# NVIDIA/nvidia-resiliency-ext

Hardware: AMD Instinct MI355X
Metric: generate_report_latency_us (lower is better)
Workload: dtype f32; 1 GPU; 8 ranks x 64 sections x 10000 samples per report, ring capacity 10000, relative+individual scores, gather_on_rank0; logical_ranks_per_gpu=8, rows_per_gpu=512, exchange=none (single process)

## Files before the change

### include/nvrx_straggler.h

```cpp
#ifndef NVRX_STRAGGLER_H
#define NVRX_STRAGGLER_H

#include <stddef.h>
#include <stdint.h>

#ifdef __cplusplus
extern "C" {
#endif

#define NVRX_ABI_VERSION 2

#define NVRX_OK 0
#define NVRX_ERR_INVALID (-22)
#define NVRX_ERR_NOMEM (-12)
#define NVRX_ERR_HIP (-5)
#define NVRX_ERR_STATE (-1)
#define NVRX_ERR_RANGE (-34)
#define NVRX_ERR_TIMEOUT (-62)

#define NVRX_STATS_STRIDE 8
#define NVRX_STAT_MIN 0
#define NVRX_STAT_MAX 1
#define NVRX_STAT_MED 2
#define NVRX_STAT_AVG 3
// ... 167 lines not shown
    int32_t stats_rows;
    double thresholds[4];
    float *d_stats;
    float *d_send;
    float *d_table;
    float *d_scores;
    uint8_t *d_flags;
    uint32_t *d_meta;
    float *d_stats_dst;
    uint32_t *d_done_counter;
    void *allgather_fn;
    void *comm;
    int32_t send_count;
    uint32_t seq;
    const uint32_t *h_seq_word;
    double timeout_s;
    void *order_after_stream;
    int32_t order_after_enabled;
    int32_t resident;
    int32_t prev_settled;
    int32_t guard_rings;
} nvrx_report_desc;
int nvrx_report(nvrx_ctx *ctx, nvrx_report_desc *desc, void *stream);
int nvrx_report_attribute(nvrx_ctx *ctx, const nvrx_report_desc *desc, int first_rank, int n_ranks, int top_n, void *d_out);
int nvrx_tail_local(nvrx_ctx *ctx, const nvrx_report_desc *desc, uint32_t q_ppm, float *d_tail_send, int K, int S,
                    int rows_active, void *stream);
int nvrx_onset_enable(nvrx_ctx *ctx, int on);
int nvrx_onset_local(nvrx_ctx *ctx, const nvrx_report_desc *desc, uint32_t min_seg_ppm, float min_strength,
                     float *d_onset_send, int K, int S, int rows_active, void *stream);
int nvrx_period_local(nvrx_ctx *ctx, const nvrx_report_desc *desc, int max_period, float min_strength,
                      float *d_period_send, int K, int S, int rows_active, void *stream);
int nvrx_episode_local(nvrx_ctx *ctx, const nvrx_report_desc *desc, uint32_t min_len_ppm, float min_strength,
                       float *d_episode_send, int K, int S, int rows_active, void *stream);
int nvrx_report_robust(nvrx_ctx *ctx, const nvrx_report_desc *desc, int first_rank, int n_ranks, int min_ranks,
                       float floor_rel, void *d_out);
int nvrx_report_peer(nvrx_ctx *ctx, const nvrx_report_desc *desc, const int32_t *d_groups, int G, int first_rank, int n_ranks,
                     int min_ranks, void *d_out);
int nvrx_report_pace(nvrx_ctx *ctx, const nvrx_report_desc *desc, int first_rank, int n_ranks, int min_ranks, void *d_out);
int nvrx_report_pace_group(nvrx_ctx *ctx, const nvrx_report_desc *desc, const int32_t *d_groups, int G, int max_group,
                           int first_rank, int n_ranks, int min_ranks, int min_peers, void *d_out);
int nvrx_report_node(nvrx_ctx *ctx, const nvrx_report_desc *desc, const int32_t *d_groups, int G, int max_group, int min_members,
                     int min_nodes, int first_rank, int n_ranks, void *d_out);
int nvrx_report_work(nvrx_ctx *ctx, const nvrx_report_desc *desc, float count_tol, int max_unlike_ppm, void *d_out);
int nvrx_report_history(nvrx_ctx *ctx, const nvrx_report_desc *desc, int first_rank, int n_ranks, float *d_hist, int S_cap,
                        int H, uint64_t n_before, const double *thresholds, void *d_out);
int nvrx_report_trend(nvrx_ctx *ctx, const float *d_hist, int n_ranks, int S, int S_cap, int H, uint64_t n_reports,
// ... 56 lines not shown
```

### nvidia-resiliency-ext_amd/csrc/nvrx_straggler.hip

```cpp
#include <hip/hip_runtime.h>
#include <hip/hip_ext.h>

#include <algorithm>
#include <atomic>
#include <chrono>
#include <thread>
#include <cmath>
#include <cstdarg>
#include <cstdio>
#include <cstdlib>
#include <cstring>
#include <deque>
#include <mutex>
#include <string>
#include <unordered_map>
#include <utility>
#include <vector>

#include "nvrx_straggler.h"

namespace {

thread_local std::string g_err;

// ... 1715 lines not shown
        uint64_t epoch;
    };
    std::vector<StreamEpoch> stream_epochs;

    const nvrx_report_desc *attr_desc = nullptr;
    hipStream_t attr_stream = nullptr;
    hipEvent_t attr_ev = nullptr;
    float *attr_scratch = nullptr;
    size_t attr_scratch_elems = 0;

    int tail_uniform_n = -1;

    bool onset_on = false;
    bool onset_wrapped = false;
    int onset_rows = 0;
    uint32_t *h_onset_starts = nullptr;
    uint32_t *d_onset_starts = nullptr;

    hipStream_t stats_stream = nullptr;
    int32_t *d_slack_list = nullptr;
    std::vector<int32_t> slack_list;
    bool slack_list_up = false;

    std::mutex mu;
};

static bool stream_is_capturing(hipStream_t st);
static void stamp_slot_give(int slot);

namespace {

int ctx_set_device(const nvrx_ctx *ctx) {
    HIP_TRY(hipSetDevice(ctx->device));
    return NVRX_OK;
}

inline void mark_side_work(nvrx_ctx *ctx) {
    ctx->side_work = true;
    ctx->side_gen++;
}

int guard_ring_writer(nvrx_ctx *ctx, hipStream_t st) {
    if (!ctx->report_epoch) return NVRX_OK;
    nvrx_ctx::StreamEpoch *se = nullptr;
    for (auto &e : ctx->stream_epochs)
        if (e.stream == st) se = &e;
// ... 1123 lines not shown
    if (!p || !p->ready || !send || !recv) return fail(NVRX_ERR_INVALID, "peer exchange is not ready");
    if (count == 0 || count > (size_t)p->stride) return fail(NVRX_ERR_RANGE, "%zu floats per rank exceed the window's %d", count, p->stride);
    *a = PeerArgs{};
    a->windows = p->d_windows;
    a->send = static_cast<const float *>(send);
    a->recv = static_cast<float *>(recv);
    a->err = p->d_err;
    a->world = p->world;
    a->rank = p->rank;
    a->count = (int)count;
    a->stride = p->stride;
    p->epoch = (p->epoch % 0x7FFFFFFFu) + 1u;
    a->epoch = p->epoch;
    a->timeout_ticks = (unsigned long long)(p->timeout_s * 1e3 * (double)p->wall_khz);
    return NVRX_OK;
}

int nvrx_report_clocks(double *out8) {
    if (!out8) return fail(NVRX_ERR_INVALID, "null argument");
    memcpy(out8, g_report_clk, sizeof(g_report_clk));
    return NVRX_OK;
}

int nvrx_report(nvrx_ctx *ctx, nvrx_report_desc *d, void *stream) {
    report_clk(0);
    if (!ctx || !d) return fail(NVRX_ERR_INVALID, "null argument");
    if (!d->d_stats || !d->d_send || !d->d_scores || !d->d_meta) return fail(NVRX_ERR_INVALID, "null buffer in the report descriptor");
    const bool exchanging = d->allgather_fn != nullptr;
    if (exchanging && (!d->d_table || d->d_table == d->d_send || d->send_count <= 0))
        return fail(NVRX_ERR_INVALID, "an exchange needs a separate table buffer and a positive send_count");
    const bool is_async = d->h_seq_word == nullptr;
    bool async_gap_ok = false;
    {
        std::lock_guard<std::mutex> lk(ctx->mu);
        const double now_us = g_report_clk[0];
        async_gap_ok = ctx->async_rehome_gap_us > 0.0 && ctx->last_report_us > 0.0 && now_us - ctx->last_report_us >= ctx->async_rehome_gap_us;
        ctx->last_report_us = now_us;
        ctx->last_rehome_verdict = 0;
        if (d->prev_settled) {
            ctx->guard_done_epoch = ctx->report_epoch;
            if (ctx->async_on_ctx && ctx->async_gen == ctx->side_gen) ctx->side_work = false;
            ctx->async_on_ctx = false;
        }
    }
    bool rehomed = false;
    if (ctx->rehome_mode && ((!is_async && !d->guard_rings) || (is_async && d->guard_rings && async_gap_ok))) {
        std::lock_guard<std::mutex> lk(ctx->mu);
        hipStream_t only = nullptr;
        int distinct = 0;
        auto see = [&](hipStream_t s) {
            if (distinct == 0 || s != only) {
                only = s;
                distinct++;
// ... 76 lines not shown
        ga.stats_out = (d->d_stats_dst && d->stats_rows > 0) ? reinterpret_cast<nvrx_f4 *>(d->d_stats_dst) : nullptr;
        ga.err = ctx->d_gather_err;
        ga.n_blocks = rows_launch;
        ga.rows_active = d->rows_active > 0 ? d->rows_active : ctx->rows_per_rank;
        ga.rows_per_rank = ctx->rows_per_rank;
        ga.local_ranks = ctx->local_ranks;
        ga.names_ok = d->names_ok ? 1.0f : 0.0f;
        ga.epoch = ctx->gran_epoch;
        ga.timeout_ticks = (unsigned long long)((d->timeout_s > 0.0 ? d->timeout_s : 1e9) * 1e3 * (double)ctx->wall_khz);
        ga.poll_naps = ctx->poll_naps;
        PeerArgs pa{};
        if (peer_route) {
            rc2 = peer_fill_args(static_cast<nvrx_peer *>(d->comm), d->d_send, d->d_table, (size_t)d->send_count, &pa);
            if (rc2) return rc2;
        }
        d->seq = (d->seq % 0x7FFFFFFFu) + 1u;
        rc2 = score_launch(exchanging ? d->d_table : d->d_send, d->R, d->K, d->S, d->do_indiv, d->do_rel, d->thresholds,
                           d->d_scores, d->d_flags, d->d_meta, d->d_done_counter, d->seq, nullptr, nullptr, 0,
                           ctx->score_stream, peer_route ? &pa : nullptr, &ga);
        if (rc2) return rc2;
        ctx->attr_desc = d, ctx->attr_stream = ctx->score_stream;
        report_clk(4);
        report_clk(5);
        rc2 = nvrx_poll_u32(d->h_seq_word, d->seq, d->timeout_s > 0.0 ? d->timeout_s : 1e30);
        report_clk(6);
        if (rc2) return rc2;
        if (*static_cast<volatile uint32_t *>(ctx->h_gather_err) == ctx->gran_epoch)
            return fail(NVRX_ERR_TIMEOUT, "the score kernel gave up waiting for the statistics kernel's rows (epoch %u)", ctx->gran_epoch);
        if (as_stream(stream) == ctx->default_stream) {
            std::lock_guard<std::mutex> lk(ctx->mu);
            ctx->side_work = false;
            ctx->async_on_ctx = false;
        }
        return NVRX_OK;
    }
    int rc = report_local_impl(ctx, d->d_stats, d->d_send, d->K, d->S, d->names_ok, d->rows_active, stream, nullptr, 0);
    if (rc) return rc;
    if (d->guard_rings) {
        std::lock_guard<std::mutex> lk(ctx->mu);
        ctx->guard_stream = as_stream(stream);
        if (rehomed || !ctx->stamps_used) {
            ctx->guard_recorded = false;
        } else {
            HIP_TRY(hipEventRecord(ctx->report_ev, as_stream(stream)));
            ctx->guard_recorded = true;
        }
        ctx->report_epoch++;
    }
    PeerArgs pa{};
    bool prologue = false;
    if (exchanging && d->allgather_fn == reinterpret_cast<void *>(&nvrx_peer_allgather) &&
        score_fits_single_wg(d->R, d->K, d->S, d->d_scores, d->d_flags) && peer_prologue_enabled()) {
        rc = peer_fill_args(static_cast<nvrx_peer *>(d->comm), d->d_send, d->d_table, (size_t)d->send_count, &pa);
        if (rc) return rc;
        prologue = true;
    } else if (exchanging) {
        using AllGatherFn = int (*)(const void *, void *, size_t, int, void *, void *);
        const int nrc = reinterpret_cast<AllGatherFn>(d->allgather_fn)(d->d_send, d->d_table, (size_t)d->send_count, 7,
                                                                       d->comm, stream);
        if (nrc != 0) {
            return fail(NVRX_ERR_HIP, "all-gather of the exchange rows failed (ncclResult %d)", nrc);
        }
    }
    report_clk(4);
    d->seq = (d->seq % 0x7FFFFFFFu) + 1u;
    rc = score_launch(exchanging ? d->d_table : d->d_send, d->R, d->K, d->S, d->do_indiv, d->do_rel, d->thresholds,
                      d->d_scores, d->d_flags, d->d_meta, d->d_done_counter, d->seq, d->d_stats, d->d_stats_dst,
                      d->stats_rows, stream, prologue ? &pa : nullptr);
    if (rc) return rc;
    ctx->attr_desc = d, ctx->attr_stream = as_stream(stream);
    report_clk(5);
    if (d->h_seq_word) {
        rc = nvrx_poll_u32(d->h_seq_word, d->seq, d->timeout_s > 0.0 ? d->timeout_s : 1e30);
        report_clk(6);
        if (rc == NVRX_OK && !rehomed && as_stream(stream) == ctx->default_stream) {
            std::lock_guard<std::mutex> lk(ctx->mu);
            ctx->side_work = false;
            ctx->async_on_ctx = false;
        }
        return rc;
    }
    if (!rehomed) {
        std::lock_guard<std::mutex> lk(ctx->mu);
        ctx->async_on_ctx = true;
        ctx->async_gen = ctx->side_gen;
    }
    return NVRX_OK;
}

static thread_local double g_window_clk[2] = {0.0, 0.0};

int nvrx_window_clocks(double *out2) {
    if (!out2) return fail(NVRX_ERR_INVALID, "out2 is null");
    out2[0] = g_window_clk[0], out2[1] = g_window_clk[1];
    return NVRX_OK;
}

int nvrx_window_report(nvrx_ctx *ctx, nvrx_report_desc *desc, void *stream, nvrx_window_desc *w) {
    if (!ctx || !desc || !w) return fail(NVRX_ERR_INVALID, "null argument");
    g_window_clk[0] = g_window_clk[1] = std::chrono::duration<double, std::micro>(std::chrono::steady_clock::now().time_since_epoch()).count();
    const bool per_kernel = w->kt_sync != nullptr;
    if (per_kernel && (!w->kt_hold || !w->kt_counter)) return fail(NVRX_ERR_INVALID, "a kernel tracer needs sync, hold and counter");
    const bool enqueue_only = w->asynchronous != 0;
    bool held = false;
    auto leave = [&](int rc) {
// ... 324 lines not shown
```

### nvidia-resiliency-ext_amd/nvrx_straggler/_native.py

```python
from __future__ import annotations

import ctypes
import os
import threading
from ctypes import POINTER, c_char_p, c_double, c_float, c_int, c_int32, c_size_t, c_uint32, c_uint64, c_void_p

_LIB_NAME = "libnvrx_straggler_hip.so"
_LIB_PATH = os.path.join(os.environ.get("NVRX_DEBUG_LIB_DIR") or os.path.join(os.path.dirname(os.path.abspath(__file__)), "lib"), _LIB_NAME)

NVRX_ABI_VERSION = 2
STATS_STRIDE = 8
STAT_MIN, STAT_MAX, STAT_MED, STAT_AVG, STAT_STD, STAT_NUM, STAT_WEIGHT = range(7)
KIND_SECTION, KIND_KERNEL = 0, 1
MAX_RING_CAP = 65536
META_WORDS = 8
ERR_TIMEOUT = -62
ERR_RANGE = -34
ERR_INVALID = -22
ERR_STATE = -1
ATTR_MAX_TOP = 16
TAIL_Q_PPM_MIN, TAIL_Q_PPM_MAX = 500000, 999999
ROUTE_SINGLE, ROUTE_ROWS, ROUTE_ROWS_PRE, ROUTE_TILE16, ROUTE_TILE8 = 1, 2, 3, 4, 5
ROBUST_MAX_RANKS = 65536
PEER_MAX_GROUPS = 4096
# ... 93 lines not shown
    ("nvrx_ring_push_staged", c_int, [c_void_p, c_void_p, c_void_p, c_int]),
    ("nvrx_sink_push", c_int, [c_void_p, c_void_p, c_void_p, c_int]),
    ("nvrx_sink_row_alloc", c_int, [c_void_p, c_int]),
    ("nvrx_ring_push_device", c_int, [c_void_p, c_int, c_void_p, c_int, c_void_p]),
    ("nvrx_ring_push_device_rows", c_int, [c_void_p, c_int, c_int, c_void_p, c_int, c_int, c_void_p]),
    ("nvrx_ring_set_count", c_int, [c_void_p, c_int, c_int]),
    ("nvrx_ring_set_count_all", c_int, [c_void_p, c_int]),
    ("nvrx_ring_count", c_int, [c_void_p, c_int]),
    ("nvrx_ring_counts", c_int, [c_void_p, c_void_p, c_int]),
    ("nvrx_ring_occupancy_changed", c_int, [c_void_p, c_int]),
    ("nvrx_window_report", c_int, [c_void_p, c_void_p, c_void_p, c_void_p]),
    ("nvrx_window_clocks", c_int, [POINTER(c_double)]),
    ("nvrx_ring_reset", c_int, [c_void_p]),
    ("nvrx_history_reset", c_int, [c_void_p, c_void_p]),
    ("nvrx_ring_flush", c_int, [c_void_p, c_void_p]),
    ("nvrx_ring_read", c_int, [c_void_p, c_int, c_void_p, c_int, c_void_p]),
    ("nvrx_event_begin", c_int, [c_void_p, c_int, c_void_p]),
    ("nvrx_event_end", c_int, [c_void_p, c_int, c_void_p]),
    ("nvrx_event_harvest", c_int, [c_void_p, c_int]),
    ("nvrx_stamp_begin", c_int, [c_void_p, c_int, c_void_p]),
    ("nvrx_stamp_end", c_int, [c_void_p, c_int, c_int, c_float, c_void_p]),
    ("nvrx_report_local", c_int, [c_void_p, c_void_p, c_void_p, c_int, c_int, c_int, c_int, c_void_p]),
    ("nvrx_report", c_int, [c_void_p, POINTER(ReportDesc), c_void_p]),
    ("nvrx_report_attribute", c_int, [c_void_p, POINTER(ReportDesc), c_int, c_int, c_int, c_void_p]),
    ("nvrx_tail_local", c_int, [c_void_p, POINTER(ReportDesc), c_uint32, c_void_p, c_int, c_int, c_int, c_void_p]),
    ("nvrx_onset_enable", c_int, [c_void_p, c_int]),
    ("nvrx_onset_local", c_int, [c_void_p, POINTER(ReportDesc), c_uint32, c_float, c_void_p, c_int, c_int, c_int, c_void_p]),
    ("nvrx_period_local", c_int, [c_void_p, POINTER(ReportDesc), c_int, c_float, c_void_p, c_int, c_int, c_int, c_void_p]),
    ("nvrx_episode_local", c_int, [c_void_p, POINTER(ReportDesc), c_uint32, c_float, c_void_p, c_int, c_int, c_int, c_void_p]),
    ("nvrx_report_robust", c_int, [c_void_p, POINTER(ReportDesc), c_int, c_int, c_int, c_float, c_void_p]),
    ("nvrx_report_peer", c_int, [c_void_p, POINTER(ReportDesc), c_void_p, c_int, c_int, c_int, c_int, c_void_p]),
    ("nvrx_report_pace", c_int, [c_void_p, POINTER(ReportDesc), c_int, c_int, c_int, c_void_p]),
    ("nvrx_report_pace_group", c_int, [c_void_p, POINTER(ReportDesc), c_void_p, c_int, c_int, c_int, c_int, c_int, c_int,
                                       c_void_p]),
    ("nvrx_report_node", c_int, [c_void_p, POINTER(ReportDesc), c_void_p, c_int, c_int, c_int, c_int, c_int, c_int, c_void_p]),
    ("nvrx_report_history", c_int, [c_void_p, POINTER(ReportDesc), c_int, c_int, c_void_p, c_int, c_int, c_uint64,
                                    POINTER(c_double), c_void_p]),
    ("nvrx_report_trend", c_int, [c_void_p, c_void_p, c_int, c_int, c_int, c_int, c_uint64, c_void_p]),
    ("nvrx_report_peer_history", c_int, [c_void_p, c_void_p, c_int, c_int, c_void_p, c_int, c_int, c_uint64, POINTER(c_double),
                                         c_void_p]),
    ("nvrx_report_peer_trend", c_int, [c_void_p, c_void_p, c_int, c_int, c_int, c_int, c_uint64, c_void_p]),
    ("nvrx_report_work", c_int, [c_void_p, POINTER(ReportDesc), c_float, c_int, c_void_p]),
    ("nvrx_slack_local", c_int, [c_void_p, POINTER(ReportDesc), c_void_p, c_void_p, c_void_p, c_int, c_void_p, c_int, c_void_p]),
    ("nvrx_report_clocks", c_int, [POINTER(c_double)]),
    ("nvrx_report_desc_size", c_int, []),
    ("nvrx_peer_create", c_int, [c_int, c_int, c_int, c_int, POINTER(c_void_p)]),
# ... 217 lines not shown
```

### nvidia-resiliency-ext_amd/nvrx_straggler/backend.py

```python
from __future__ import annotations

import ctypes
import os
import threading
import weakref
from typing import Any, Dict, List, Optional, Sequence

import numpy as np
import torch

from . import _native
from .row_families import EPISODE, FAMILIES, ONSET, PERIOD, TAIL, RowFamily
from .table_families import NODE, PACE, PACE_GROUP, PEER, ROBUST, SLOTS, TableFamily

DEFAULT_THRESHOLDS = (0.75, 0.75, 0.75, 0.75)



def report_timeout_s() -> float:
    t = _timeout_cache[0]
    if t is None:
        t = refresh_report_timeout()
    return t

# ... 1391 lines not shown
                                        rows_active, self.backend.stream_handle)
        if rc < 0:
            _native.check(rc)

    @staticmethod
    def configure_desc(ws: Workspace, blk: ResultBlock, key: tuple) -> None:
        rows_active, stats_rows, do_indiv, do_rel, thresholds, direct, names_ok, wait, resident = key
        d = blk.desc
        d.rows_active, d.stats_rows = rows_active, min(stats_rows, ws.stats_rows)
        d.do_indiv, d.do_rel = int(do_indiv), int(do_rel)
        d.names_ok = int(names_ok)
        for i in range(4):
            d.thresholds[i] = float(thresholds[i])
        if direct is not None:
            d.allgather_fn, d.comm = direct.fn_address, direct.comm_address
        else:
            d.allgather_fn, d.comm = None, None
        d.timeout_s = report_timeout_s()
        d.h_seq_word = blk.h_seq if wait else None
        d.guard_rings = 0 if wait else 1
        d.resident = 1 if (wait and resident) else 0
        blk.desc_key = key

    def report_fused(self, ws: Workspace, rows_active: int, stats_rows: int, do_indiv: bool, do_rel: bool,
                     thresholds: Sequence[float], direct=None, names_ok: bool = True, wait: bool = True,
                     order_after: Optional[int] = None, resident: bool = True, prev_settled: bool = False) -> int:
        blk = ws.flip()
        d = blk.desc
        key = (rows_active, stats_rows, do_indiv, do_rel, thresholds, direct, names_ok, wait, resident)
        if blk.desc_key != key:
            self.configure_desc(ws, blk, key)
        d.prev_settled = 1 if (prev_settled and not wait) else 0
        if order_after is not None:
            d.order_after_stream, d.order_after_enabled = order_after, 1
        elif d.order_after_enabled:
            d.order_after_enabled = 0
        if not ws.send_initialised:
            self.backend.send_init(ws)
            self.backend.synchronize()
        d.seq = ws.seq
        rc = self.lib.nvrx_report(self.ctx, blk.desc_ref, self.backend._stream_handle)
        ws.seq = d.seq
        if rc < 0:
            if rc == _native.ERR_TIMEOUT:
                self.backend.retire_workspace(ws)
            _native.check(rc)
        return ws.seq

    def report_attribute(self, ws: Workspace, top_n: int, first_rank: int = 0, n_ranks: Optional[int] = None) -> Attribution:
        n_ranks = ws.R - first_rank if n_ranks is None else n_ranks
        ws.attr_settle()
        buf, _ = ws.attr_buffers(n_ranks, top_n, False)
        rc = self.lib.nvrx_report_attribute(self.ctx, ws.block.desc_ref, first_rank, n_ranks, top_n, buf.data_ptr())
        if rc < 0:
            _native.check(rc)
        out = ws._attr_last = Attribution(self.backend, buf, first_rank, n_ranks, top_n)
        return out

    def _table_report(self, fam: TableFamily, ws: Workspace, groups: Optional[PeerGroups], first_rank: int,
                      n_ranks: Optional[int], params: tuple) -> TableScores:
        return self.backend._table_step(fam, ws, getattr(self.lib, fam.c_report), (self.ctx, ws.block.desc_ref), (), groups,
                                        first_rank, n_ranks, params)

    def report_robust(self, ws: Workspace, first_rank: int = 0, n_ranks: Optional[int] = None, min_ranks: int = 4,
                      floor_rel: float = 0.02) -> TableScores:
        return self._table_report(ROBUST, ws, None, first_rank, n_ranks, (min_ranks, floor_rel))

    def report_peer(self, ws: Workspace, groups: PeerGroups, first_rank: int = 0, n_ranks: Optional[int] = None,
                    min_ranks: int = 2) -> TableScores:
        return self._table_report(PEER, ws, groups, first_rank, n_ranks, (min_ranks,))
# ... 119 lines not shown
```

### nvidia-resiliency-ext_amd/nvrx_straggler/folded.py

```python
from __future__ import annotations

from typing import Optional, Sequence

import numpy as np
import torch

from . import _native, dist_utils
from .backend import get_backend
from .reporting import ReportGenerator


class FoldedJob:
    def __init__(self, total_ranks: int = 8, section_names: Optional[Sequence[str]] = None, sections: int = 64,
                 ring_cap: int = 8192, scores_to_compute=("relative_perf_scores", "individual_perf_scores"),
                 gather_on_rank0: bool = True, pg=None, node_name: str = "node", kernel_attribution: int = 0,
                 tail_quantile: float = 0.0, robust_scores: bool = False, asynchronous: bool = False,
                 onset_detection: bool = False, onset_min_segment: float = 0.05, onset_min_strength: float = 0.5,
                 period_detection: bool = False, period_max: int = 1024, period_min_strength: float = 0.5,
                 episode_detection: bool = False, episode_min_length: float = 0.005, episode_min_strength: float = 0.5,
                 score_history: int = 0, persistence_min_reports: int = 3, persistence_thresholds=None,
                 score_trends: bool = False, trend_min_reports: int = 6, trend_min_tau: float = 0.6, trend_horizon=None,
                 collective_slack: bool = False, slack_min_ranks: int = 4, slack_min_share: float = 0.05,
                 slack_max_ratio: float = 0.25, kernel_names: Sequence[str] = (), peer_groups=None, peer_min_ranks: int = 2,
                 pace_scores: bool = False, pace_min_ranks: int = 4, pace_min_columns: int = 8, pace_min_effect: float = 0.03,
# ... 53 lines not shown
        return range(self.world_rank * self.local_ranks, (self.world_rank + 1) * self.local_ranks)

    def load(self, lr: int, samples) -> None:
        if isinstance(samples, np.ndarray):
            samples = torch.from_numpy(np.ascontiguousarray(samples, dtype=np.float32)).to(self.backend.device)
        self.backend.synchronize()
        torch.cuda.current_stream().synchronize()
        rows = [self.rows[name] for name in self.section_names]
        if rows == list(range(rows[0], rows[0] + len(rows))) and samples.dim() == 2 and samples.stride(1) == 1:
            self.rings.push_device_rows(rows[0], samples, lr=lr)
        else:
            for s, row in enumerate(rows):
                self.rings.push_device(row, samples[s].contiguous(), lr=lr)
        self.backend.synchronize()

    def load_kernels(self, lr: int, samples) -> None:
        for name, values in zip(self.kernel_names, samples):
            self.rings.push_many(self._no_kernel_rows[name], values, lr=lr)

    def rearm(self, n: int) -> None:
        self.rings.set_count_all(n)

    def report(self, reset: bool = True):
        rep = self.reporter.generate_report_from_rings(self.rings, self.rows, self._no_kernel_rows,
                                                       local_ranks=self.local_ranks)
        if reset:
            self.rings.reset()
        return rep

    def close(self) -> None:
        self.reporter.close()
        self.rings.close()
```

### nvidia-resiliency-ext_amd/nvrx_straggler/reporting.py

```python
from __future__ import annotations

import collections
import dataclasses
import itertools
import logging
import math
import os
import threading
import time
from typing import Any, Dict, List, Mapping, Optional, Sequence

import numpy as np

from . import backend as _backend_mod
from . import dist_utils, row_families
from .name_mapper import NameMapper, name_digest
from .statistics import NUM_COLUMN, STAT_KEYS, Statistic

_SummaryType = Mapping[Statistic, float]
_LOG = logging.getLogger(__name__)



def _load_pyread():
# ... 1596 lines not shown
        self.world_size = dist_utils.get_world_size(self.group)
        self.rank = dist_utils.get_rank(self.group)
        self.node_name = node_name
        self.thresholds = tuple(float(t) for t in thresholds)

        self.min_local_kernel_times: Dict[str, float] = collections.defaultdict(lambda: float("inf"))
        self.min_local_section_times: Dict[str, float] = collections.defaultdict(lambda: float("inf"))

        self.name_mapper = NameMapper(pg=pg)
        self._private_mapper = NameMapper(pg=pg)
        self.rank_to_node: Dict[int, str] = collections.defaultdict(lambda: "<unk>")
        self._rank_to_node_folded = False
        self._direct = None
        self._direct_tried = False
        self.asynchronous = bool(asynchronous)
        self.exchange_info: Dict[str, Any] = {}
        self._ring_plan = None
        self._ring_gid_state = None
        self._inflight: Optional[_PendingBlock] = None
        self._prev_async_settled = True
        self._resync_pending = False
        self._had_ring_report = False
        self._unreported_rows: list = []
        n = int(kernel_attribution)
        if not 0 <= n <= 16:
            raise ValueError(f"kernel_attribution must be 0 (off) or 1..16 kernels per GPU score, got {kernel_attribution!r}")
        self.kernel_attribution = n
        if n:
            be = _backend_mod._backend
            if be is not None and not hasattr(be, "attribute"):
                raise RuntimeError(f"kernel_attribution={n}: the active backend ({getattr(be, 'name', type(be).__name__)}) "
                                   "has no kernel attribution (backend.attribute)")
        self._attr_names_cache = (None, 0, ())
        self.tail_q_ppm = _backend_mod._native.tail_q_ppm(tail_quantile)
        if self.tail_q_ppm:
            if not self.is_computing_rel_scores:
                raise ValueError(f"tail_quantile={tail_quantile!r} needs relative_perf_scores among scores_to_compute "
                                 f"(got {scores_to_compute!r}): tail scores are relative scores")
            be = _backend_mod._backend
            if be is not None and not hasattr(be, "tail_score"):
                raise RuntimeError(f"tail_quantile={tail_quantile!r}: the active backend ({getattr(be, 'name', type(be).__name__)}) "
                                   "has no tail scores (backend.tail_score)")
        self.robust_scores = bool(robust_scores)
        if self.robust_scores:
            if isinstance(robust_min_ranks, bool) or not isinstance(robust_min_ranks, (int, np.integer)) or robust_min_ranks < 1:
                raise ValueError(f"robust_min_ranks must be an integer >= 1, got {robust_min_ranks!r}")
# ... 603 lines not shown
            return False
        self._inflight = None
        names_word = pend.complete()
        self._prev_async_settled = True
        self._check_exchange()
        return names_word != 1

    def _drop_plan(self) -> None:
        self._ring_plan = None

    def _sync_names_first(self) -> None:
        self._ring_plan = None
        self._resync_pending = True

    def _take_resync(self) -> bool:
        pending, self._resync_pending = self._resync_pending, False
        return pending

    def _check_exchange(self) -> None:
        check = getattr(self._direct, "check", None)
        if check is not None:
            check()

    def _report_from_plan(self, plan, rings, t0, order_after=None, names_ok: bool = True):
        be = _backend_mod.get_backend()
        ws = plan.ws
        multi = self.world_size > 1 and self._exchanged()
        fused = plan.fused and (not multi or self._direct is not None)
        attr_n = self.kernel_attribution
        settle = getattr(ws, "settle_readers", None)
        if settle is not None:
            settle()
        self._last_plan_fused = fused
        if fused and attr_n and not hasattr(rings, "report_attribute"):
            raise RuntimeError(f"kernel_attribution={attr_n}: these rings run the one-call report but have no report_attribute")
        if fused and self.robust_scores and not hasattr(rings, "report_robust"):
            raise RuntimeError("robust_scores: these rings run the one-call report but have no report_robust")
        if fused and self.work_groups and not hasattr(rings, "report_work"):
            raise RuntimeError("work_groups: these rings run the one-call report but have no report_work")
        if fused and self.peer_groups is not None and not hasattr(rings, "report_peer"):
            raise RuntimeError("peer_groups: these rings run the one-call report but have no report_peer")
        if fused and self.pace_scores and not hasattr(rings, "report_pace_group" if self.pace_peer_groups else "report_pace"):
            if self.pace_peer_groups:
                raise RuntimeError("pace_peer_groups: these rings run the one-call report but have no report_pace_group")
            raise RuntimeError("pace_scores: these rings run the one-call report but have no report_pace")
        if fused and self.node_scores and not hasattr(rings, "report_node"):
            raise RuntimeError("node_scores: these rings run the one-call report but have no report_node")
        if fused and self._peer_history is not None and not hasattr(rings, "report_peer_history"):
            raise RuntimeError("peer_history: these rings run the one-call report but have no report_peer_history")
        if fused and self.peer_trends and not hasattr(rings, "report_peer_trend"):
            raise RuntimeError("peer_trends: these rings run the one-call report but have no report_peer_trend")
        if fused and self._history is not None and not hasattr(rings, "report_history"):
            raise RuntimeError("score_history: these rings run the one-call report but have no report_history")
        if fused and self.score_trends and not hasattr(rings, "report_trend"):
            raise RuntimeError("score_trends: these rings run the one-call report but have no report_trend")
        if fused:
            wait = not self.asynchronous
            seq = rings.report_fused(ws, plan.rows_used, plan.stats_needed, self.is_computing_indiv_scores,
                                     self.is_computing_rel_scores, self.thresholds, self._direct if multi else None,
                                     names_ok=names_ok, wait=wait, order_after=order_after if multi else None,
                                     resident=not (multi and getattr(self._direct, "shared_device", False)
                                                   and os.environ.get("NVRX_DEBUG_RESIDENT_SHARED_OK", "0") in ("", "0")),
                                     prev_settled=self._prev_async_settled)
            if not wait:
                self._prev_async_settled = False
                pend = self._inflight = _PendingBlock(be, ws, seq)
                if self.gather_on_rank0 and self.rank != 0:
                    return None
                report = Report._from_device(
                    _ScoreSource(plan.view, pend),
                    self._shared_rank_to_node(),
                    (time.perf_counter_ns() - t0) * 1e-6, self.gather_on_rank0, self.rank)
                if attr_n:
                    self._attach_plan_attribution(report, plan, rings, True)
                if self.robust_scores:
                    self._attach_plan_robust(report, plan, rings, True)
                if self.work_groups:
                    self._attach_plan_work(report, plan, rings, True)
                if self.peer_groups is not None:
                    self._attach_plan_peer(report, plan, rings, True)
# ... 24 lines not shown
            ws.attach(pending)
        else:
            pending = ws.host_block()
        report = Report._from_device(
            _ScoreSource(plan.view, pending),
            self._shared_rank_to_node(),
            (time.perf_counter_ns() - t0) * 1e-6, self.gather_on_rank0, self.rank)
        if attr_n:
            self._attach_plan_attribution(report, plan, rings, fused)
        if self.robust_scores:
            self._attach_plan_robust(report, plan, rings, fused)
        if self.work_groups:
            self._attach_plan_work(report, plan, rings, fused)
        if self.peer_groups is not None:
            self._attach_plan_peer(report, plan, rings, fused)
        if self.pace_scores:
            self._attach_plan_pace(report, plan, rings, fused)
        if self.node_scores:
            self._attach_plan_node(report, plan, rings, fused)
        if self._history is not None:
            self._attach_plan_history(report, plan, rings, fused)
        return report

    def _attach_plan_attribution(self, report, plan, rings, fused: bool) -> None:
        ws = plan.ws
        lo, hi = plan.view.layout[5], plan.view.layout[6]
        if fused:
            handle = rings.report_attribute(ws, self.kernel_attribution, lo, hi - lo)
        else:
            handle = _backend_mod.get_backend().attribute(ws, ws.table, self.kernel_attribution, self.is_computing_indiv_scores,
                                                          self.is_computing_rel_scores, lo, hi - lo)
        report.__dict__["_attr"] = self._attr_source(handle, ws, plan.mapper, lo, hi, plan.view.ranks)

    def _robust_min(self, ws) -> int:
        return min(self.robust_min_ranks, ws.R)

    def _attach_robust(self, report, handle, ws, mapper, view) -> None:
        report.__dict__["_robust"] = _RobustSource(handle, view.ranks, view.cols, self._attr_names(mapper, ws.K),
                                                   self._robust_min(ws), self.robust_floor)

    def _attach_plan_robust(self, report, plan, rings, fused: bool) -> None:
        ws = plan.ws
        lo, hi = plan.view.layout[5], plan.view.layout[6]
        if fused:
            handle = rings.report_robust(ws, lo, hi - lo, self._robust_min(ws), self.robust_floor)
        else:
# ... 254 lines not shown
            row = np.zeros(L, dtype=np.float32)
            row[:KS] = -1.0
            row[KS : 2 * KS] = np.nan
            for name, summ in kernel_summaries.items():
                g = mapper.kernel_name_to_id.get(name)
                if g is None:
                    continue
                row[g] = summ[Statistic.MED]
                row[KS + g] = self.min_local_kernel_times[name] if self.is_computing_indiv_scores else np.nan
                row[2 * KS + g] = summ[Statistic.NUM] * summ[Statistic.AVG]
            for name, summ in section_summaries.items():
                g = mapper.section_name_to_id.get(name)
                if g is None:
                    continue
                row[K + g] = summ[Statistic.MED]
                row[KS + K + g] = self.min_local_section_times[name] if self.is_computing_indiv_scores else np.nan
            row[L - 1] = 1.0 if names_ok else 0.0
            ws.set_send_row(0, row)

        ws, mapper = self._score_round(knames, snames, fill_send)
        return self._assemble(ws, mapper, snames, section_summaries, kernel_summaries, t0)

    def generate_report_from_rings(self, rings, section_rows: Mapping[str, int], kernel_rows: Mapping[str, int],
                                   local_ranks: int = 1, order_after: Optional[int] = None):
        t0 = time.perf_counter_ns()
        self.world_size, self.rank = dist_utils.world_and_rank(self.group, self._wr_cache)
        if self._starts_family is not None and not getattr(rings, "onset_enabled", False):
            if not hasattr(rings, "onset_enable"):
                raise RuntimeError(f"{self._starts_family.option}: the active backend has no ring-start snapshot (rings.onset_enable)")
            rings.onset_enable(True)
        if not self._direct_tried and self.world_size != 1:
            self._maybe_create_direct_exchange()
        if self._inflight is not None and self._settle_inflight():
            self._sync_names_first()
        if self._resync_pending:
            self._ring_plan = None
        plan = self._ring_plan
        if plan is not None and plan.key == self._plan_key(rings, section_rows, kernel_rows, local_ranks):
            try:
                out = self._report_from_plan(plan, rings, t0, order_after)
            except Exception:
                self._drop_plan()
                raise
            if out is not False:
                self._family_steps(out, rings, plan.ws, plan.mapper, plan.rows_used, self._last_plan_fused, local_ranks)
                if self.collective_slack:
                    self._slack_step(out, rings, plan.ws, plan.rows_used, self._last_plan_fused, local_ranks)
                return out
            self._sync_names_first()
        elif (plan is not None and self.enqueue_only() and plan.fused and plan.topology == self._plan_topology(rings, local_ranks)
              and not plan.mapper.has_all_names(list(kernel_rows.keys()), list(section_rows.keys()))):
            known_k, known_s = plan.kernel_rows, plan.section_rows
            self._unreported_rows = ([r for n, r in kernel_rows.items() if n not in known_k and not is_collective_kernel(n)]
                                     + [r for n, r in section_rows.items() if n not in known_s])
            out = self._report_from_plan(plan, rings, t0, order_after, names_ok=False)
            self._family_steps(out, rings, plan.ws, plan.mapper, plan.rows_used, self._last_plan_fused, local_ranks)
            if self.collective_slack:
                self._slack_step(out, rings, plan.ws, plan.rows_used, self._last_plan_fused, local_ranks)
            return out
        kernel_rows = {k: r for k, r in kernel_rows.items() if not is_collective_kernel(k)} if any(
            is_collective_kernel(k) for k in kernel_rows) else kernel_rows
        self._maybe_gather_rank_to_node()
        if local_ranks > 1 and not self._rank_to_node_folded:
            per_proc = dict(self.rank_to_node)
            self.rank_to_node = {p * local_ranks + q: node for p, node in per_proc.items() for q in range(local_ranks)}
            self._rank_to_node_folded = True
        knames, snames = list(kernel_rows.keys()), list(section_rows.keys())
        rows_used = rings.rows_used
        total_rows = rings.local_ranks * rings.rows_per_rank
        stats_needed = rows_used

        def fill_send(ws, mapper, names_ok):
            state = (id(mapper), mapper.version, rows_used, id(ws))
            if self._ring_gid_state != state:
                self._point_ring_rows(rings, mapper, ws)
                self._ring_gid_state = state
            rings.report_local(ws, names_ok, rows_active=rows_used)

        not_the_first, self._had_ring_report = self._had_ring_report, True
        ws, mapper = self._score_round(knames, snames, fill_send, local_ranks=local_ranks, stats_rows=total_rows,
                                       stats_rows_used=stats_needed, sync_first=self._take_resync(), may_defer_sync=not_the_first)
        report = self._assemble(ws, mapper, snames, dict(section_rows), dict(kernel_rows), t0, local_ranks=local_ranks,
                                stats=ws.stats[:stats_needed].copy())
        self._family_steps(report, rings, ws, mapper, rows_used, False, local_ranks)
        if self.collective_slack:
            self._slack_step(report, rings, ws, rows_used, False, local_ranks)
        self._ring_plan = self._build_ring_plan(self._plan_key(rings, section_rows, kernel_rows, local_ranks), rings,
                                                section_rows, kernel_rows, local_ranks)
        return report
```

Before: 27.55 us.

## Split fused report into issue and wait to overlap host work with GPU

Splits nvrx_report into nvrx_report_issue and nvrx_report_wait, so the Python side enqueues the score kernel, then builds the report object and resets the rings while the GPU runs, and only afterwards polls the completion word. The goal is to hide host-side assembly and ring-reset overhead behind kernel execution in the synchronous single-process path. In exchange it adds pending-report state on the context, more control flow in the reporting path, and a ring reset that is reordered relative to the wait.

```diff
diff --git a/include/nvrx_straggler.h b/include/nvrx_straggler.h
--- a/include/nvrx_straggler.h
+++ b/include/nvrx_straggler.h
@@ -213,6 +213,8 @@
     int32_t guard_rings;
 } nvrx_report_desc;
 int nvrx_report(nvrx_ctx *ctx, nvrx_report_desc *desc, void *stream);
+int nvrx_report_issue(nvrx_ctx *ctx, nvrx_report_desc *desc, void *stream);
+int nvrx_report_wait(nvrx_ctx *ctx, nvrx_report_desc *desc);
 int nvrx_report_attribute(nvrx_ctx *ctx, const nvrx_report_desc *desc, int first_rank, int n_ranks, int top_n, void *d_out);
 int nvrx_tail_local(nvrx_ctx *ctx, const nvrx_report_desc *desc, uint32_t q_ppm, float *d_tail_send, int K, int S,
                     int rows_active, void *stream);
diff --git a/nvidia-resiliency-ext_amd/csrc/nvrx_straggler.hip b/nvidia-resiliency-ext_amd/csrc/nvrx_straggler.hip
--- a/nvidia-resiliency-ext_amd/csrc/nvrx_straggler.hip
+++ b/nvidia-resiliency-ext_amd/csrc/nvrx_straggler.hip
@@ -1761,6 +1761,14 @@
     std::vector<int32_t> slack_list;
     bool slack_list_up = false;
 
+    struct PendingReport {
+        nvrx_report_desc *desc = nullptr;
+        uint32_t seq = 0, gran_epoch = 0;
+        bool resident = false, rehomed = false;
+        hipStream_t stream = nullptr;
+        uint64_t side_gen = 0;
+    } pending_report;
+
     std::mutex mu;
 };
 
@@ -2930,13 +2938,16 @@
     return NVRX_OK;
 }
 
-int nvrx_report(nvrx_ctx *ctx, nvrx_report_desc *d, void *stream) {
-    report_clk(0);
+static int report_check_args(const nvrx_ctx *ctx, const nvrx_report_desc *d) {
     if (!ctx || !d) return fail(NVRX_ERR_INVALID, "null argument");
     if (!d->d_stats || !d->d_send || !d->d_scores || !d->d_meta) return fail(NVRX_ERR_INVALID, "null buffer in the report descriptor");
+    if (d->allgather_fn != nullptr && (!d->d_table || d->d_table == d->d_send || d->send_count <= 0))
+        return fail(NVRX_ERR_INVALID, "an exchange needs a separate table buffer and a positive send_count");
+    return NVRX_OK;
+}
+
+static int report_enqueue(nvrx_ctx *ctx, nvrx_report_desc *d, void *stream, nvrx_ctx::PendingReport *out) {
     const bool exchanging = d->allgather_fn != nullptr;
-    if (exchanging && (!d->d_table || d->d_table == d->d_send || d->send_count <= 0))
-        return fail(NVRX_ERR_INVALID, "an exchange needs a separate table buffer and a positive send_count");
     const bool is_async = d->h_seq_word == nullptr;
     bool async_gap_ok = false;
     {
@@ -3059,16 +3070,7 @@
         ctx->attr_desc = d, ctx->attr_stream = ctx->score_stream;
         report_clk(4);
         report_clk(5);
-        rc2 = nvrx_poll_u32(d->h_seq_word, d->seq, d->timeout_s > 0.0 ? d->timeout_s : 1e30);
-        report_clk(6);
-        if (rc2) return rc2;
-        if (*static_cast<volatile uint32_t *>(ctx->h_gather_err) == ctx->gran_epoch)
-            return fail(NVRX_ERR_TIMEOUT, "the score kernel gave up waiting for the statistics kernel's rows (epoch %u)", ctx->gran_epoch);
-        if (as_stream(stream) == ctx->default_stream) {
-            std::lock_guard<std::mutex> lk(ctx->mu);
-            ctx->side_work = false;
-            ctx->async_on_ctx = false;
-        }
+        out->resident = true, out->rehomed = rehomed, out->stream = as_stream(stream), out->gran_epoch = ctx->gran_epoch;
         return NVRX_OK;
     }
     int rc = report_local_impl(ctx, d->d_stats, d->d_send, d->K, d->S, d->names_ok, d->rows_active, stream, nullptr, 0);
@@ -3107,17 +3109,65 @@
     if (rc) return rc;
     ctx->attr_desc = d, ctx->attr_stream = as_stream(stream);
     report_clk(5);
-    if (d->h_seq_word) {
-        rc = nvrx_poll_u32(d->h_seq_word, d->seq, d->timeout_s > 0.0 ? d->timeout_s : 1e30);
-        report_clk(6);
-        if (rc == NVRX_OK && !rehomed && as_stream(stream) == ctx->default_stream) {
-            std::lock_guard<std::mutex> lk(ctx->mu);
-            ctx->side_work = false;
-            ctx->async_on_ctx = false;
-        }
-        return rc;
-    }
-    if (!rehomed) {
+    out->resident = false, out->rehomed = rehomed, out->stream = as_stream(stream), out->gran_epoch = 0;
+    return NVRX_OK;
+}
+
+int nvrx_report_issue(nvrx_ctx *ctx, nvrx_report_desc *d, void *stream) {
+    report_clk(0);
+    int rc = report_check_args(ctx, d);
+    if (rc) return rc;
+    if (!d->h_seq_word)
+        return fail(NVRX_ERR_INVALID, "nvrx_report_issue needs a completion word (h_seq_word): asynchronous reports go through nvrx_report");
+    if (ctx->pending_report.desc) return fail(NVRX_ERR_STATE, "a report is pending on this context: nvrx_report_wait comes first");
+    nvrx_ctx::PendingReport p;
+    {
+        std::lock_guard<std::mutex> lk(ctx->mu);
+        p.side_gen = ctx->side_gen;
+    }
+    rc = report_enqueue(ctx, d, stream, &p);
+    if (rc) return rc;
+    p.desc = d, p.seq = d->seq;
+    ctx->pending_report = p;
+    return NVRX_OK;
+}
+
+int nvrx_report_wait(nvrx_ctx *ctx, nvrx_report_desc *d) {
+    if (!ctx || !d) return fail(NVRX_ERR_INVALID, "null argument");
+    if (!ctx->pending_report.desc) return fail(NVRX_ERR_STATE, "no report is pending on this context");
+    const nvrx_ctx::PendingReport p = ctx->pending_report;
+    ctx->pending_report = nvrx_ctx::PendingReport();
+    if (p.desc != d) return fail(NVRX_ERR_STATE, "the report pending on this context was issued through another descriptor");
+    const int rc = nvrx_poll_u32(d->h_seq_word, p.seq, d->timeout_s > 0.0 ? d->timeout_s : 1e30);
+    report_clk(6);
+    if (rc) return rc;
+    if (p.resident) {
+        if (*static_cast<volatile uint32_t *>(ctx->h_gather_err) == p.gran_epoch)
+            return fail(NVRX_ERR_TIMEOUT, "the score kernel gave up waiting for the statistics kernel's rows (epoch %u)", p.gran_epoch);
+        if (p.stream != ctx->default_stream) return NVRX_OK;
+    } else if (p.rehomed || p.stream != ctx->default_stream) {
+        return NVRX_OK;
+    }
+    std::lock_guard<std::mutex> lk(ctx->mu);
+    if (ctx->side_gen == p.side_gen) {
+        ctx->side_work = false;
+        ctx->async_on_ctx = false;
+    }
+    return NVRX_OK;
+}
+
+int nvrx_report(nvrx_ctx *ctx, nvrx_report_desc *d, void *stream) {
+    if (ctx && d && d->h_seq_word) {
+        const int rc = nvrx_report_issue(ctx, d, stream);
+        return rc ? rc : nvrx_report_wait(ctx, d);
+    }
+    report_clk(0);
+    int rc = report_check_args(ctx, d);
+    if (rc) return rc;
+    nvrx_ctx::PendingReport p;
+    rc = report_enqueue(ctx, d, stream, &p);
+    if (rc) return rc;
+    if (!p.rehomed) {
         std::lock_guard<std::mutex> lk(ctx->mu);
         ctx->async_on_ctx = true;
         ctx->async_gen = ctx->side_gen;
diff --git a/nvidia-resiliency-ext_amd/csrc/report_split_args_check.cpp b/nvidia-resiliency-ext_amd/csrc/report_split_args_check.cpp
--- /dev/null
+++ b/nvidia-resiliency-ext_amd/csrc/report_split_args_check.cpp
@@ -0,0 +1,63 @@
+#include "args_check.h"
+
+int main() {
+    nvrx_ctx *ctx = reinterpret_cast<nvrx_ctx *>(uintptr_t{4096});
+    uint32_t word = 0;
+    nvrx_report_desc good;
+    memset(&good, 0, sizeof(good));
+    good.R = 2, good.K = 0, good.S = 4, good.names_ok = 1, good.do_indiv = good.do_rel = 1;
+    good.d_stats = reinterpret_cast<float *>(uintptr_t{8192});
+    good.d_send = reinterpret_cast<float *>(uintptr_t{12288});
+    good.d_table = reinterpret_cast<float *>(uintptr_t{16384});
+    good.d_scores = reinterpret_cast<float *>(uintptr_t{20480});
+    good.d_flags = reinterpret_cast<uint8_t *>(uintptr_t{24576});
+    good.d_meta = reinterpret_cast<uint32_t *>(uintptr_t{28672});
+    good.h_seq_word = &word;
+    good.seq = 7;
+    void *gather = reinterpret_cast<void *>(uintptr_t{32768});
+
+    nvrx_report_desc d = good;
+    expect("issue: null context", nvrx_report_issue(nullptr, &d, nullptr), NVRX_ERR_INVALID, "null argument");
+    expect("issue: null descriptor", nvrx_report_issue(ctx, nullptr, nullptr), NVRX_ERR_INVALID, "null argument");
+    expect("issue: both null", nvrx_report_issue(nullptr, nullptr, nullptr), NVRX_ERR_INVALID, "null argument");
+    d = good, d.d_stats = nullptr;
+    expect("issue: null statistics", nvrx_report_issue(ctx, &d, nullptr), NVRX_ERR_INVALID, "null buffer");
+    d = good, d.d_send = nullptr;
+    expect("issue: null exchange rows", nvrx_report_issue(ctx, &d, nullptr), NVRX_ERR_INVALID, "null buffer");
+    d = good, d.d_scores = nullptr;
+    expect("issue: null scores", nvrx_report_issue(ctx, &d, nullptr), NVRX_ERR_INVALID, "null buffer");
+    d = good, d.d_meta = nullptr;
+    expect("issue: null meta", nvrx_report_issue(ctx, &d, nullptr), NVRX_ERR_INVALID, "null buffer");
+    d = good, d.allgather_fn = gather, d.send_count = 16, d.d_table = nullptr;
+    expect("issue: exchange without a table", nvrx_report_issue(ctx, &d, nullptr), NVRX_ERR_INVALID, "separate table");
+    d = good, d.allgather_fn = gather, d.send_count = 16, d.d_table = d.d_send;
+    expect("issue: exchange into its own rows", nvrx_report_issue(ctx, &d, nullptr), NVRX_ERR_INVALID, "separate table");
+    d = good, d.allgather_fn = gather, d.send_count = 0;
+    expect("issue: exchange of nothing", nvrx_report_issue(ctx, &d, nullptr), NVRX_ERR_INVALID, "send_count");
+    d = good, d.h_seq_word = nullptr;
+    expect("issue: no completion word", nvrx_report_issue(ctx, &d, nullptr), NVRX_ERR_INVALID, "h_seq_word");
+    d = good, d.h_seq_word = nullptr, d.d_meta = nullptr;
+    expect("issue: null buffer before the word", nvrx_report_issue(ctx, &d, nullptr), NVRX_ERR_INVALID, "null buffer");
+    d = good, d.d_scores = nullptr;
+    (void)nvrx_report_issue(ctx, &d, nullptr);
+    if (d.seq != good.seq) {
+        fprintf(stderr, "FAIL a refused issue moved desc.seq from %u to %u\n", good.seq, d.seq);
+        failures++;
+    }
+
+    d = good;
+    expect("wait: null context", nvrx_report_wait(nullptr, &d), NVRX_ERR_INVALID, "null argument");
+    expect("wait: null descriptor", nvrx_report_wait(ctx, nullptr), NVRX_ERR_INVALID, "null argument");
+    expect("wait: both null", nvrx_report_wait(nullptr, nullptr), NVRX_ERR_INVALID, "null argument");
+
+    expect("report: null context", nvrx_report(nullptr, &d, nullptr), NVRX_ERR_INVALID, "null argument");
+    expect("report: null descriptor", nvrx_report(ctx, nullptr, nullptr), NVRX_ERR_INVALID, "null argument");
+    d = good, d.d_send = nullptr;
+    expect("report: null buffer, synchronous", nvrx_report(ctx, &d, nullptr), NVRX_ERR_INVALID, "null buffer");
+    d = good, d.h_seq_word = nullptr, d.d_send = nullptr;
+    expect("report: null buffer, asynchronous", nvrx_report(ctx, &d, nullptr), NVRX_ERR_INVALID, "null buffer");
+    d = good, d.allgather_fn = gather, d.send_count = 16, d.d_table = nullptr;
+    expect("report: exchange without a table", nvrx_report(ctx, &d, nullptr), NVRX_ERR_INVALID, "separate table");
+    printf("report_split_args_check: %d failure(s)\n", failures);
+    return failures ? 1 : 0;
+}
diff --git a/nvidia-resiliency-ext_amd/nvrx_straggler/_native.py b/nvidia-resiliency-ext_amd/nvrx_straggler/_native.py
--- a/nvidia-resiliency-ext_amd/nvrx_straggler/_native.py
+++ b/nvidia-resiliency-ext_amd/nvrx_straggler/_native.py
@@ -139,6 +139,8 @@
     ("nvrx_stamp_end", c_int, [c_void_p, c_int, c_int, c_float, c_void_p]),
     ("nvrx_report_local", c_int, [c_void_p, c_void_p, c_void_p, c_int, c_int, c_int, c_int, c_void_p]),
     ("nvrx_report", c_int, [c_void_p, POINTER(ReportDesc), c_void_p]),
+    ("nvrx_report_issue", c_int, [c_void_p, POINTER(ReportDesc), c_void_p]),
+    ("nvrx_report_wait", c_int, [c_void_p, POINTER(ReportDesc)]),
     ("nvrx_report_attribute", c_int, [c_void_p, POINTER(ReportDesc), c_int, c_int, c_int, c_void_p]),
     ("nvrx_tail_local", c_int, [c_void_p, POINTER(ReportDesc), c_uint32, c_void_p, c_int, c_int, c_int, c_void_p]),
     ("nvrx_onset_enable", c_int, [c_void_p, c_int]),
diff --git a/nvidia-resiliency-ext_amd/nvrx_straggler/backend.py b/nvidia-resiliency-ext_amd/nvrx_straggler/backend.py
--- a/nvidia-resiliency-ext_amd/nvrx_straggler/backend.py
+++ b/nvidia-resiliency-ext_amd/nvrx_straggler/backend.py
@@ -1437,9 +1437,9 @@
         d.resident = 1 if (wait and resident) else 0
         blk.desc_key = key
 
-    def report_fused(self, ws: Workspace, rows_active: int, stats_rows: int, do_indiv: bool, do_rel: bool,
-                     thresholds: Sequence[float], direct=None, names_ok: bool = True, wait: bool = True,
-                     order_after: Optional[int] = None, resident: bool = True, prev_settled: bool = False) -> int:
+    def _report_prepare(self, ws: Workspace, rows_active: int, stats_rows: int, do_indiv: bool, do_rel: bool,
+                        thresholds: Sequence[float], direct, names_ok: bool, wait: bool, order_after: Optional[int],
+                        resident: bool, prev_settled: bool) -> ResultBlock:
         blk = ws.flip()
         d = blk.desc
         key = (rows_active, stats_rows, do_indiv, do_rel, thresholds, direct, names_ok, wait, resident)
@@ -1454,13 +1454,39 @@
             self.backend.send_init(ws)
             self.backend.synchronize()
         d.seq = ws.seq
+        return blk
+
+    def report_fused(self, ws: Workspace, rows_active: int, stats_rows: int, do_indiv: bool, do_rel: bool,
+                     thresholds: Sequence[float], direct=None, names_ok: bool = True, wait: bool = True,
+                     order_after: Optional[int] = None, resident: bool = True, prev_settled: bool = False) -> int:
+        blk = self._report_prepare(ws, rows_active, stats_rows, do_indiv, do_rel, thresholds, direct, names_ok, wait,
+                                   order_after, resident, prev_settled)
         rc = self.lib.nvrx_report(self.ctx, blk.desc_ref, self.backend._stream_handle)
-        ws.seq = d.seq
+        ws.seq = blk.desc.seq
         if rc < 0:
             if rc == _native.ERR_TIMEOUT:
                 self.backend.retire_workspace(ws)
             _native.check(rc)
         return ws.seq
+
+    def report_issue(self, ws: Workspace, rows_active: int, stats_rows: int, do_indiv: bool, do_rel: bool,
+                     thresholds: Sequence[float], direct=None, names_ok: bool = True, order_after: Optional[int] = None,
+                     resident: bool = True) -> int:
+        blk = self._report_prepare(ws, rows_active, stats_rows, do_indiv, do_rel, thresholds, direct, names_ok, True,
+                                   order_after, resident, False)
+        rc = self.lib.nvrx_report_issue(self.ctx, blk.desc_ref, self.backend._stream_handle)
+        ws.seq = blk.desc.seq
+        if rc < 0:
+            _native.check(rc)
+        return ws.seq
+
+    def report_wait(self, ws: Workspace) -> None:
+        rc = self.lib.nvrx_report_wait(self.ctx, ws.block.desc_ref)
+        if rc < 0:
+            ws.block._live = None
+            if rc == _native.ERR_TIMEOUT:
+                self.backend.retire_workspace(ws)
+            _native.check(rc)
 
     def report_attribute(self, ws: Workspace, top_n: int, first_rank: int = 0, n_ranks: Optional[int] = None) -> Attribution:
         n_ranks = ws.R - first_rank if n_ranks is None else n_ranks
diff --git a/nvidia-resiliency-ext_amd/nvrx_straggler/folded.py b/nvidia-resiliency-ext_amd/nvrx_straggler/folded.py
--- a/nvidia-resiliency-ext_amd/nvrx_straggler/folded.py
+++ b/nvidia-resiliency-ext_amd/nvrx_straggler/folded.py
@@ -99,11 +99,8 @@
         self.rings.set_count_all(n)
 
     def report(self, reset: bool = True):
-        rep = self.reporter.generate_report_from_rings(self.rings, self.rows, self._no_kernel_rows,
-                                                       local_ranks=self.local_ranks)
-        if reset:
-            self.rings.reset()
-        return rep
+        return self.reporter.generate_report_from_rings(self.rings, self.rows, self._no_kernel_rows,
+                                                        local_ranks=self.local_ranks, reset_rings=reset)
 
     def close(self) -> None:
         self.reporter.close()
diff --git a/nvidia-resiliency-ext_amd/nvrx_straggler/reporting.py b/nvidia-resiliency-ext_amd/nvrx_straggler/reporting.py
--- a/nvidia-resiliency-ext_amd/nvrx_straggler/reporting.py
+++ b/nvidia-resiliency-ext_amd/nvrx_straggler/reporting.py
@@ -1642,6 +1642,8 @@
         self._resync_pending = False
         self._had_ring_report = False
         self._unreported_rows: list = []
+        self._report_split = os.environ.get("NVRX_DEBUG_REPORT_SPLIT", "1") != "0"
+        self._rings_were_reset = False
         n = int(kernel_attribution)
         if not 0 <= n <= 16:
             raise ValueError(f"kernel_attribution must be 0 (off) or 1..16 kernels per GPU score, got {kernel_attribution!r}")
@@ -2291,7 +2293,7 @@
         if check is not None:
             check()
 
-    def _report_from_plan(self, plan, rings, t0, order_after=None, names_ok: bool = True):
+    def _report_from_plan(self, plan, rings, t0, order_after=None, names_ok: bool = True, reset_rings: bool = False):
         be = _backend_mod.get_backend()
         ws = plan.ws
         multi = self.world_size > 1 and self._exchanged()
@@ -2325,6 +2327,10 @@
             raise RuntimeError("score_trends: these rings run the one-call report but have no report_trend")
         if fused:
             wait = not self.asynchronous
+            if wait and not multi and self._report_split:
+                issue = getattr(rings, "report_issue", None)
+                if issue is not None:
+                    return self._report_split_from_plan(plan, rings, be, t0, issue, names_ok, reset_rings)
             seq = rings.report_fused(ws, plan.rows_used, plan.stats_needed, self.is_computing_indiv_scores,
                                      self.is_computing_rel_scores, self.thresholds, self._direct if multi else None,
                                      names_ok=names_ok, wait=wait, order_after=order_after if multi else None,
@@ -2395,6 +2401,44 @@
             self._attach_plan_history(report, plan, rings, fused)
         return report
 
+    def _report_split_from_plan(self, plan, rings, be, t0, issue, names_ok: bool, reset_rings: bool):
+        ws = plan.ws
+        seq = issue(ws, plan.rows_used, plan.stats_needed, self.is_computing_indiv_scores, self.is_computing_rel_scores,
+                    self.thresholds, None, names_ok=names_ok, order_after=None, resident=True)
+        report = None
+        if not (self.gather_on_rank0 and self.rank != 0):
+            pending = _LiveBlock(be, ws, seq, plan.stats_needed)
+            ws.attach(pending)
+            report = Report._from_device(_ScoreSource(plan.view, pending), self._shared_rank_to_node(), 0.0,
+                                         self.gather_on_rank0, self.rank)
+        if reset_rings and not self._row_families and not self.collective_slack:
+            rings.reset()
+            self._rings_were_reset = True
+        rings.report_wait(ws)
+        if report is None or ws.meta[0] != 1:
+            mark = getattr(ws, "mark_live", None)
+            if mark is not None:
+                mark(seq)
+            if ws.meta[0] != 1:
+                return False
+            return None
+        report.__dict__["generate_report_elapsed_time"] = (time.perf_counter_ns() - t0) * 1e-6
+        if self.kernel_attribution:
+            self._attach_plan_attribution(report, plan, rings, True)
+        if self.robust_scores:
+            self._attach_plan_robust(report, plan, rings, True)
+        if self.work_groups:
+            self._attach_plan_work(report, plan, rings, True)
+        if self.peer_groups is not None:
+            self._attach_plan_peer(report, plan, rings, True)
+        if self.pace_scores:
+            self._attach_plan_pace(report, plan, rings, True)
+        if self.node_scores:
+            self._attach_plan_node(report, plan, rings, True)
+        if self._history is not None:
+            self._attach_plan_history(report, plan, rings, True)
+        return report
+
     def _attach_plan_attribution(self, report, plan, rings, fused: bool) -> None:
         ws = plan.ws
         lo, hi = plan.view.layout[5], plan.view.layout[6]
@@ -2695,7 +2739,7 @@
         return self._assemble(ws, mapper, snames, section_summaries, kernel_summaries, t0)
 
     def generate_report_from_rings(self, rings, section_rows: Mapping[str, int], kernel_rows: Mapping[str, int],
-                                   local_ranks: int = 1, order_after: Optional[int] = None):
+                                   local_ranks: int = 1, order_after: Optional[int] = None, reset_rings: bool = False):
         t0 = time.perf_counter_ns()
         self.world_size, self.rank = dist_utils.world_and_rank(self.group, self._wr_cache)
         if self._starts_family is not None and not getattr(rings, "onset_enabled", False):
@@ -2711,15 +2755,22 @@
         plan = self._ring_plan
         if plan is not None and plan.key == self._plan_key(rings, section_rows, kernel_rows, local_ranks):
             try:
-                out = self._report_from_plan(plan, rings, t0, order_after)
+                out = self._report_from_plan(plan, rings, t0, order_after, True, reset_rings)
             except Exception:
+                self._rings_were_reset = False
                 self._drop_plan()
                 raise
             if out is not False:
                 self._family_steps(out, rings, plan.ws, plan.mapper, plan.rows_used, self._last_plan_fused, local_ranks)
                 if self.collective_slack:
                     self._slack_step(out, rings, plan.ws, plan.rows_used, self._last_plan_fused, local_ranks)
+                if reset_rings:
+                    if self._rings_were_reset:
+                        self._rings_were_reset = False
+                    else:
+                        rings.reset()
                 return out
+            self._rings_were_reset = False
             self._sync_names_first()
         elif (plan is not None and self.enqueue_only() and plan.fused and plan.topology == self._plan_topology(rings, local_ranks)
               and not plan.mapper.has_all_names(list(kernel_rows.keys()), list(section_rows.keys()))):
@@ -2730,6 +2781,8 @@
             self._family_steps(out, rings, plan.ws, plan.mapper, plan.rows_used, self._last_plan_fused, local_ranks)
             if self.collective_slack:
                 self._slack_step(out, rings, plan.ws, plan.rows_used, self._last_plan_fused, local_ranks)
+            if reset_rings:
+                rings.reset()
             return out
         kernel_rows = {k: r for k, r in kernel_rows.items() if not is_collective_kernel(k)} if any(
             is_collective_kernel(k) for k in kernel_rows) else kernel_rows
@@ -2760,4 +2813,6 @@
             self._slack_step(report, rings, ws, rows_used, False, local_ranks)
         self._ring_plan = self._build_ring_plan(self._plan_key(rings, section_rows, kernel_rows, local_ranks), rings,
                                                 section_rows, kernel_rows, local_ranks)
+        if reset_rings:
+            rings.reset()
         return report
```

After: 26.13 us, median of 6. 5.2% less time.
